# somepago/DCR

Hardware: NVIDIA H100
Metric: embed+top-k query images/sec (higher is better)
Workload: dtype bf16

## Files before the change

dcr_b200/csrc/stem_fused.cu:

```cuda
#include <cuda_bf16.h>

#include <algorithm>
#include <cstring>

#include "dcr_internal.cuh"
#include "host_util.cuh"
#include "ptx.cuh"

namespace dcr {

namespace {

constexpr int kSN = 64;
constexpr int kSTile = 512;
constexpr int kSBlocks = kSTile / 128;
constexpr int kSThreads = 288;
constexpr int kWBytes = kSN * 256 * 2;

struct StemParams {
  const __nv_bfloat16* planes;
  long long img_stride;
  long long plane_stride;
  int B, OH, OW, PW;
  int units_per_img, tiles_per_unit, num_units;
  int part_rows;
  int OHp, OWp, prow_per_part;
  int win_units;
  int win_stages;
  int ring_rows;
  const float* scale;
  const float* bias;
  __nv_bfloat16* out;
};

DCR_DEVICE uint64_t desc_nosw(uint32_t addr) {
  uint64_t d = 0;
  d |= static_cast<uint64_t>((addr & 0x3FFFF) >> 4);
  d |= static_cast<uint64_t>(16 >> 4) << 16;
  d |= static_cast<uint64_t>(256 >> 4) << 32;
  return d;
}

DCR_DEVICE void bulk_load(void* dst, const void* src, uint32_t bytes, uint64_t* bar) {
  asm volatile("cp.async.bulk.shared::cluster.global.mbarrier::complete_tx::bytes [%0], [%1], %2, [%3];" ::"r"(smem_u32(dst)),
               "l"(reinterpret_cast<uint64_t>(src)), "r"(bytes), "r"(smem_u32(bar))
               : "memory");
}

DCR_DEVICE int unit_begin(const StemParams& p, int part, bool pool) {
  if (!pool) return part * kSTile;
  const int row_lo = max(0, part * p.part_rows - 1);
  return row_lo * p.PW;
}

template <bool kPool>
__global__ void __launch_bounds__(kSThreads, 1) stem_conv_kernel(const __grid_constant__ CUtensorMap tmap_w, const StemParams p) {
  extern __shared__ __align__(1024) uint8_t smem_raw[];
  uint8_t* smem = smem_align1024(smem_raw);
  const int win_bytes = p.win_units * 16;
  const int stage_bytes = (2 * win_bytes + 1023) & ~1023;
  uint8_t* s_w = smem;
  uint8_t* s_win = s_w + kWBytes;
  uint8_t* s_out = s_win + p.win_stages * stage_bytes;
  const int ring_row_bytes = p.OW * 128;
  const int ring_mask = p.ring_rows - 1;
  uint8_t* acc_xpose = s_out + (kPool ? ((p.ring_rows * ring_row_bytes + 1023) & ~1023) : 2 * 16384);
  float* sb = reinterpret_cast<float*>(acc_xpose + 8 * kAccXposeWarpBytes);
  uint64_t* bars = reinterpret_cast<uint64_t*>(sb + 128);
  uint64_t* w_full = bars;
  uint64_t* win_full = bars + 1;
  uint64_t* win_empty = bars + 5;

  const uint32_t warp = threadIdx.x >> 5, lane = threadIdx.x & 31;
  if (warp == 8 && lane == 0) tma_prefetch_desc(&tmap_w);
  if (warp == 0 && lane == 0) {
    mbar_init(w_full, 1);
    for (int s = 0; s < 4; ++s) {
      mbar_init(&win_full[s], 1);
      mbar_init(&win_empty[s], 8);
    }
    fence_mbar_init();
  }
  __syncthreads();

  if (warp == 8) {
    if (elect_one()) {
      mbar_arrive_expect_tx(w_full, kWBytes);
      for (int kb = 0; kb < 4; ++kb) tma_load_2d(s_w + kb * 8192, &tmap_w, w_full, kb * 64, 0, kEvictLast);
    }
    __syncwarp();
    PipeState ws(p.win_stages);
    for (int unit = blockIdx.x; unit < p.num_units; unit += gridDim.x) {
      const int b = unit / p.units_per_img;
      const int mu = unit_begin(p, unit - b * p.units_per_img, kPool);
      for (int t = 0; t < p.tiles_per_unit; ++t, ws.next()) {
        const int m0 = mu + t * kSTile;
        mbar_wait(&win_empty[ws.s], ws.ph ^ 1);
        if (elect_one()) {
          mbar_arrive_expect_tx(&win_full[ws.s], 2 * win_bytes);
          const __nv_bfloat16* src = p.planes + static_cast<size_t>(b) * p.img_stride + static_cast<size_t>(m0) * 8;
          bulk_load(s_win + ws.s * stage_bytes, src, win_bytes, &win_full[ws.s]);
          bulk_load(s_win + ws.s * stage_bytes + win_bytes, src + p.plane_stride, win_bytes, &win_full[ws.s]);
        }
        __syncwarp();
      }
    }
  } else {
    const uint32_t ewarp = warp;
    const uint32_t quad = warp & 3;
    const uint32_t half = ewarp >> 2;
    const uint32_t row = quad * 32 + lane;
    const uint32_t etid = ewarp * 32 + lane;
    const uint32_t xacc = smem_u32(acc_xpose) + warp * kAccXposeWarpBytes;
    const uint32_t win0 = smem_u32(s_win);
    const uint32_t PW = static_cast<uint32_t>(p.PW);
    const uint64_t dw0 = wgmma_desc_sw128(smem_u32(s_w) + half * 32 * 128);
    PipeState ws(p.win_stages);
    const uint32_t sb_addr = smem_u32(sb), so_addr = smem_u32(s_out);
    for (int c = etid; c < kSN; c += 256) {
      st_shared_f32(sb_addr + c * 4, p.scale ? p.scale[c] : 1.f);
      st_shared_f32(sb_addr + (kSN + c) * 4, p.bias ? p.bias[c] : 0.f);
    }
    asm volatile("bar.sync 1, 256;" ::: "memory");
    float sc[32], bi[32];
#pragma unroll
    for (int c = 0; c < 32; c += 4) {
      const float4 s4 = ld_shared_f4(sb_addr + (half * 32 + c) * 4);
      const float4 b4 = ld_shared_f4(sb_addr + (kSN + half * 32 + c) * 4);
      sc[c] = s4.x; sc[c + 1] = s4.y; sc[c + 2] = s4.z; sc[c + 3] = s4.w;
      bi[c] = b4.x; bi[c + 1] = b4.y; bi[c + 2] = b4.z; bi[c + 3] = b4.w;
    }
    const int positions = p.OH * p.PW;
    mbar_wait(w_full, 0);
    uint32_t tc = 0, blk = 0;
    for (int unit = blockIdx.x; unit < p.num_units; unit += gridDim.x) {
      const int b = unit / p.units_per_img;
      const int part = unit - b * p.units_per_img;
      const int mu = unit_begin(p, part, kPool);
      const int row_lo = kPool ? max(0, part * p.part_rows - 1) : 0;
      const int row_hi = kPool ? min(p.OH, (part + 1) * p.part_rows) : p.OH;
      int next_yp = part * p.prow_per_part;
      const int yp_end = min(p.OHp, next_yp + p.prow_per_part);
      if constexpr (kPool) asm volatile("bar.sync 2, 256;" ::: "memory");
      for (int t = 0; t < p.tiles_per_unit; ++t, ++tc, ws.next()) {
        const int m0 = mu + t * kSTile;
        mbar_wait(&win_full[ws.s], ws.ph);
        const uint32_t wbase = win0 + ws.s * stage_bytes;
#pragma unroll 1
        for (int mb = 0; mb < kSBlocks; ++mb, ++blk) {
          WgAcc<32> acc;
          wgmma_fence();
#pragma unroll
          for (int a = 0; a < 4; ++a) {
#pragma unroll
            for (int e = 0; e < 2; ++e) {
#pragma unroll
              for (int bp = 0; bp < 2; ++bp) {
                const uint32_t a_addr = wbase + e * win_bytes + (mb * 128 + a * PW + 2 * bp) * 16;
                const int kc = (a * 2 + e) * 2 + bp;
                const uint64_t db = dw0 + static_cast<uint64_t>((kc >> 2) * (8192 >> 4) + (kc & 3) * 2);
                acc.mma2(desc_nosw(a_addr), desc_nosw(a_addr + 128), db, kc != 0);
              }
            }
          }
          wgmma_commit();
          wgmma_wait<0>();
          acc.fence_regs();
          if (mb == kSBlocks - 1 && lane == 0) mbar_arrive(&win_empty[ws.s]);
          uint32_t r[32];
          acc.rows32(0, r, xacc, lane);
          uint4 v[4];
#pragma unroll
          for (int q = 0; q < 4; ++q) {
            v[q].x = pack_bf16x2(fmaxf(fmaf(__uint_as_float(r[q * 8 + 0]), sc[q * 8 + 0], bi[q * 8 + 0]), 0.f),
                                 fmaxf(fmaf(__uint_as_float(r[q * 8 + 1]), sc[q * 8 + 1], bi[q * 8 + 1]), 0.f));
            v[q].y = pack_bf16x2(fmaxf(fmaf(__uint_as_float(r[q * 8 + 2]), sc[q * 8 + 2], bi[q * 8 + 2]), 0.f),
                                 fmaxf(fmaf(__uint_as_float(r[q * 8 + 3]), sc[q * 8 + 3], bi[q * 8 + 3]), 0.f));
            v[q].z = pack_bf16x2(fmaxf(fmaf(__uint_as_float(r[q * 8 + 4]), sc[q * 8 + 4], bi[q * 8 + 4]), 0.f),
                                 fmaxf(fmaf(__uint_as_float(r[q * 8 + 5]), sc[q * 8 + 5], bi[q * 8 + 5]), 0.f));
            v[q].w = pack_bf16x2(fmaxf(fmaf(__uint_as_float(r[q * 8 + 6]), sc[q * 8 + 6], bi[q * 8 + 6]), 0.f),
                                 fmaxf(fmaf(__uint_as_float(r[q * 8 + 7]), sc[q * 8 + 7], bi[q * 8 + 7]), 0.f));
          }
          const int mblk = m0 + mb * 128;
          if constexpr (!kPool) {
            const uint32_t stage = so_addr + (blk & 1) * 16384;
            const uint32_t srow = stage + row * 128;
            const uint32_t sw = row & 7;
#pragma unroll
            for (int q = 0; q < 4; ++q) st_shared_v4(srow + (((half * 4 + q) ^ sw) << 4), v[q]);
            asm volatile("bar.sync 2, 256;" ::: "memory");
#pragma unroll
            for (int it = 0; it < 4; ++it) {
              const int pos = it * 32 + static_cast<int>(etid >> 3);
              const int ch16 = static_cast<int>(etid & 7);
              const int m = mblk + pos;
              const int y = m / p.PW, x = m - y * p.PW;
              if (m < positions && x < p.OW) {
                const uint4 o = ld_shared_v4(stage + pos * 128 + ((ch16 ^ (pos & 7)) << 4));
                __nv_bfloat16* dst = p.out + ((static_cast<size_t>(b) * p.OH + y) * p.OW + x) * kSN + ch16 * 8;
                *reinterpret_cast<uint4*>(dst) = o;
              }
            }
          } else {
            const int m = mblk + static_cast<int>(row);
            const int y = m / p.PW, x = m - y * p.PW;
            if (x < p.OW && y >= row_lo && y < row_hi) {
              const uint32_t rrow = so_addr + (y & ring_mask) * ring_row_bytes + x * 128;
#pragma unroll
              for (int q = 0; q < 4; ++q) st_shared_v4(rrow + (((half * 4 + q) ^ (x & 7)) << 4), v[q]);
            }
            asm volatile("bar.sync 2, 256;" ::: "memory");
            const int yc = min((mblk + 128) / p.PW - 1, row_hi - 1);
            while (next_yp < yp_end && min(2 * next_yp + 1, p.OH - 1) <= yc) {
              const int y1 = 2 * next_yp;
              const uint32_t r0 = so_addr + (max(y1 - 1, 0) & ring_mask) * ring_row_bytes;
              const uint32_t r1 = so_addr + (y1 & ring_mask) * ring_row_bytes;
              const uint32_t r2 = so_addr + (min(y1 + 1, p.OH - 1) & ring_mask) * ring_row_bytes;
              for (int idx = etid; idx < p.OWp * 8; idx += 256) {
                const int xp = idx >> 3, c = idx & 7;
                const int x1 = 2 * xp, x0 = max(x1 - 1, 0), x2 = min(x1 + 1, p.OW - 1);
                const uint32_t o0 = x0 * 128 + ((c ^ (x0 & 7)) << 4), o1 = x1 * 128 + ((c ^ (x1 & 7)) << 4),
                               o2 = x2 * 128 + ((c ^ (x2 & 7)) << 4);
                uint4 w[9];
                w[0] = ld_shared_v4(r0 + o0); w[1] = ld_shared_v4(r0 + o1); w[2] = ld_shared_v4(r0 + o2);
                w[3] = ld_shared_v4(r1 + o0); w[4] = ld_shared_v4(r1 + o1); w[5] = ld_shared_v4(r1 + o2);
                w[6] = ld_shared_v4(r2 + o0); w[7] = ld_shared_v4(r2 + o1); w[8] = ld_shared_v4(r2 + o2);
                uint4 o;
                {
                  auto mx = [](uint32_t a, uint32_t b) {
                    __nv_bfloat162 r = __hmax2(*reinterpret_cast<const __nv_bfloat162*>(&a), *reinterpret_cast<const __nv_bfloat162*>(&b));
                    return *reinterpret_cast<uint32_t*>(&r);
                  };
                  auto mx9 = [&](auto get) {
                    const uint32_t a = mx(mx(get(w[0]), get(w[1])), mx(get(w[2]), get(w[3])));
                    const uint32_t b = mx(mx(get(w[4]), get(w[5])), mx(get(w[6]), get(w[7])));
                    return mx(mx(a, b), get(w[8]));
                  };
                  o.x = mx9([](const uint4& v) { return v.x; });
                  o.y = mx9([](const uint4& v) { return v.y; });
                  o.z = mx9([](const uint4& v) { return v.z; });
                  o.w = mx9([](const uint4& v) { return v.w; });
                }
                __nv_bfloat16* dst = p.out + ((static_cast<size_t>(b) * p.OHp + next_yp) * p.OWp + xp) * kSN + c * 8;
                *reinterpret_cast<uint4*>(dst) = o;
              }
              ++next_yp;
            }
          }
        }
      }
    }
  }

}

int stem_ring_rows(int PW) {
  int r = 8;
  while (r < 255 / PW + 4) r *= 2;
  return r;
}

}

int stem_fused_pitch(int out_w) { return out_w + 4; }
long long stem_fused_plane_units(int out_h, int out_w) {
  const int PW = stem_fused_pitch(out_w);
  const long long tiles = (static_cast<long long>(out_h) * PW + kSTile - 1) / kSTile;
  return tiles * kSTile + 3ll * PW + 16 + 2 * kSTile;
}

int stem_conv(const __nv_bfloat16* planes, int B, int OH, int OW, const __nv_bfloat16* weight, const float* scale, const float* bias,
              __nv_bfloat16* out, cudaStream_t stream, int pool) {
  const DeviceInfo* di = device_info();
  if (!di) return -2;
  if (int rc = require_sm90a(di, "stem_conv")) return rc;
  if (B == 0) return 0;
  StemParams p;
  memset(&p, 0, sizeof(p));
  p.planes = planes; p.B = B; p.OH = OH; p.OW = OW;
  p.PW = stem_fused_pitch(OW);
  p.plane_stride = stem_fused_plane_units(OH, OW) * 8;
  p.img_stride = 2 * p.plane_stride;
  const int tiles_per_img = static_cast<int>((static_cast<long long>(OH) * p.PW + kSTile - 1) / kSTile);
  p.win_units = (kSTile + 3 * p.PW + 3 + 7) & ~7;
  p.scale = scale; p.bias = bias; p.out = out;
  p.OHp = (OH - 1) / 2 + 1;
  p.OWp = (OW - 1) / 2 + 1;
  p.ring_rows = stem_ring_rows(p.PW);
  if (pool) {
    const int parts = (p.OHp % 4 == 0) ? 4 : ((p.OHp % 2 == 0) ? 2 : 1);
    p.units_per_img = parts;
    p.prow_per_part = p.OHp / parts;
    p.part_rows = 2 * p.prow_per_part;
    p.tiles_per_unit = static_cast<int>((static_cast<long long>(p.part_rows + 1) * p.PW + kSTile - 1) / kSTile);
    const long long last_unit = static_cast<long long>(std::max(0, (parts - 1) * p.part_rows - 1)) * p.PW;
    DCR_REQUIRE(last_unit + static_cast<long long>(p.tiles_per_unit) * kSTile + 3ll * p.PW + 8 <= stem_fused_plane_units(OH, OW),
                "stem_conv: plane slack too small for the pooled schedule (%d x %d)", OH, OW);
  } else {
    p.units_per_img = tiles_per_img;
    p.tiles_per_unit = 1;
    p.prow_per_part = 0;
    p.part_rows = 0;
  }
  p.num_units = B * p.units_per_img;
  CUtensorMap tw;
  if (int rc = make_tmap_2d_bf16(&tw, weight, kSN, 256, 256, kSN, 64)) return rc;
  const size_t stage = (static_cast<size_t>(2) * p.win_units * 16 + 1023) & ~size_t(1023);
  const size_t out_bytes = pool ? ((static_cast<size_t>(p.ring_rows) * OW * 128 + 1023) & ~size_t(1023)) : 2 * 16384;
  const size_t fixed = 1024 + kWBytes + out_bytes + 8 * kAccXposeWarpBytes + 512 + 256;
  DCR_REQUIRE(fixed + stage <= di->max_smem_optin, "stem_conv: image too wide for the window buffers (OW = %d)", OW);
  p.win_stages = static_cast<int>(std::min<size_t>(4, (di->max_smem_optin - fixed) / stage));
  const size_t smem = fixed + p.win_stages * stage;
  const int grid = std::min(p.num_units, di->num_sms);
  return launch(pool ? stem_conv_kernel<true> : stem_conv_kernel<false>, grid, kSThreads, smem, stream, "stem_conv", tw, p);
}

}
```

Baseline: 3459.

## Ping-pong two consumer warpgroups over full-width stem conv blocks

```diff
diff --git a/dcr_b200/csrc/stem_fused.cu b/dcr_b200/csrc/stem_fused.cu
--- a/dcr_b200/csrc/stem_fused.cu
+++ b/dcr_b200/csrc/stem_fused.cu
@@ -14,8 +14,11 @@
 constexpr int kSN = 64;
 constexpr int kSTile = 512;
 constexpr int kSBlocks = kSTile / 128;
-constexpr int kSThreads = 288;
+constexpr int kSThreads = 384;
+constexpr int kSConsumerRegs = 224, kSProducerRegs = 56;
 constexpr int kWBytes = kSN * 256 * 2;
+constexpr int kStageBytes = 128 * 128;
+constexpr int kSPoolMaxOW = 131;
 
 struct StemParams {
   const __nv_bfloat16* planes;
@@ -64,12 +67,13 @@
   uint8_t* s_out = s_win + p.win_stages * stage_bytes;
   const int ring_row_bytes = p.OW * 128;
   const int ring_mask = p.ring_rows - 1;
-  uint8_t* acc_xpose = s_out + (kPool ? ((p.ring_rows * ring_row_bytes + 1023) & ~1023) : 2 * 16384);
-  float* sb = reinterpret_cast<float*>(acc_xpose + 8 * kAccXposeWarpBytes);
-  uint64_t* bars = reinterpret_cast<uint64_t*>(sb + 128);
+  float* sb = reinterpret_cast<float*>(s_out + (kPool ? ((p.ring_rows * ring_row_bytes + 1023) & ~1023) : 2 * kStageBytes));
+  uint64_t* bars = reinterpret_cast<uint64_t*>(sb + 2 * kSN);
   uint64_t* w_full = bars;
   uint64_t* win_full = bars + 1;
   uint64_t* win_empty = bars + 5;
+  uint64_t* turn = bars + 9;
+  uint64_t* stored = bars + 11;
 
   const uint32_t warp = threadIdx.x >> 5, lane = threadIdx.x & 31;
   if (warp == 8 && lane == 0) tma_prefetch_desc(&tmap_w);
@@ -79,60 +83,67 @@
       mbar_init(&win_full[s], 1);
       mbar_init(&win_empty[s], 8);
     }
+    for (int g = 0; g < 2; ++g) {
+      mbar_init(&turn[g], 4);
+      mbar_init(&stored[g], 4);
+    }
     fence_mbar_init();
   }
   __syncthreads();
 
-  if (warp == 8) {
-    if (elect_one()) {
-      mbar_arrive_expect_tx(w_full, kWBytes);
-      for (int kb = 0; kb < 4; ++kb) tma_load_2d(s_w + kb * 8192, &tmap_w, w_full, kb * 64, 0, kEvictLast);
-    }
-    __syncwarp();
-    PipeState ws(p.win_stages);
-    for (int unit = blockIdx.x; unit < p.num_units; unit += gridDim.x) {
-      const int b = unit / p.units_per_img;
-      const int mu = unit_begin(p, unit - b * p.units_per_img, kPool);
-      for (int t = 0; t < p.tiles_per_unit; ++t, ws.next()) {
-        const int m0 = mu + t * kSTile;
-        mbar_wait(&win_empty[ws.s], ws.ph ^ 1);
-        if (elect_one()) {
-          mbar_arrive_expect_tx(&win_full[ws.s], 2 * win_bytes);
-          const __nv_bfloat16* src = p.planes + static_cast<size_t>(b) * p.img_stride + static_cast<size_t>(m0) * 8;
-          bulk_load(s_win + ws.s * stage_bytes, src, win_bytes, &win_full[ws.s]);
-          bulk_load(s_win + ws.s * stage_bytes + win_bytes, src + p.plane_stride, win_bytes, &win_full[ws.s]);
+  if (warp >= 8) {
+    wg_regs_dec<kSProducerRegs>();
+    if (warp == 8) {
+      if (elect_one()) {
+        mbar_arrive_expect_tx(w_full, kWBytes);
+        for (int kb = 0; kb < 4; ++kb) tma_load_2d(s_w + kb * 8192, &tmap_w, w_full, kb * 64, 0, kEvictLast);
+      }
+      __syncwarp();
+      PipeState ws(p.win_stages);
+      for (int unit = blockIdx.x; unit < p.num_units; unit += gridDim.x) {
+        const int b = unit / p.units_per_img;
+        const int mu = unit_begin(p, unit - b * p.units_per_img, kPool);
+        for (int t = 0; t < p.tiles_per_unit; ++t, ws.next()) {
+          const int m0 = mu + t * kSTile;
+          mbar_wait(&win_empty[ws.s], ws.ph ^ 1);
+          if (elect_one()) {
+            mbar_arrive_expect_tx(&win_full[ws.s], 2 * win_bytes);
+            const __nv_bfloat16* src = p.planes + static_cast<size_t>(b) * p.img_stride + static_cast<size_t>(m0) * 8;
+            bulk_load(s_win + ws.s * stage_bytes, src, win_bytes, &win_full[ws.s]);
+            bulk_load(s_win + ws.s * stage_bytes + win_bytes, src + p.plane_stride, win_bytes, &win_full[ws.s]);
+          }
+          __syncwarp();
         }
-        __syncwarp();
       }
     }
   } else {
-    const uint32_t ewarp = warp;
+    wg_regs_inc<kSConsumerRegs>();
+    const uint32_t wg = warp >> 2;
     const uint32_t quad = warp & 3;
-    const uint32_t half = ewarp >> 2;
-    const uint32_t row = quad * 32 + lane;
-    const uint32_t etid = ewarp * 32 + lane;
-    const uint32_t xacc = smem_u32(acc_xpose) + warp * kAccXposeWarpBytes;
+    const uint32_t gtid = quad * 32 + lane;
+    const uint32_t r0 = lane >> 2, c0 = 2 * (lane & 3);
     const uint32_t win0 = smem_u32(s_win);
     const uint32_t PW = static_cast<uint32_t>(p.PW);
-    const uint64_t dw0 = wgmma_desc_sw128(smem_u32(s_w) + half * 32 * 128);
-    PipeState ws(p.win_stages);
+    const uint64_t dw0 = wgmma_desc_sw128(smem_u32(s_w));
     const uint32_t sb_addr = smem_u32(sb), so_addr = smem_u32(s_out);
-    for (int c = etid; c < kSN; c += 256) {
+    for (int c = warp * 32 + lane; c < kSN; c += 256) {
       st_shared_f32(sb_addr + c * 4, p.scale ? p.scale[c] : 1.f);
       st_shared_f32(sb_addr + (kSN + c) * 4, p.bias ? p.bias[c] : 0.f);
     }
-    asm volatile("bar.sync 1, 256;" ::: "memory");
-    float sc[32], bi[32];
-#pragma unroll
-    for (int c = 0; c < 32; c += 4) {
-      const float4 s4 = ld_shared_f4(sb_addr + (half * 32 + c) * 4);
-      const float4 b4 = ld_shared_f4(sb_addr + (kSN + half * 32 + c) * 4);
-      sc[c] = s4.x; sc[c + 1] = s4.y; sc[c + 2] = s4.z; sc[c + 3] = s4.w;
-      bi[c] = b4.x; bi[c + 1] = b4.y; bi[c + 2] = b4.z; bi[c + 3] = b4.w;
+    named_bar_sync(1, 256);
+    float2 sc[8], bi[8];
+#pragma unroll
+    for (int j = 0; j < 8; ++j) {
+      sc[j] = ld_shared_f2(sb_addr + (8 * j + c0) * 4);
+      bi[j] = ld_shared_f2(sb_addr + (kSN + 8 * j + c0) * 4);
     }
     const int positions = p.OH * p.PW;
+    const PingPong pingpong{turn};
+    const PingPong ring_order{stored};
+    const uint32_t stage_addr = so_addr + wg * kStageBytes;
     mbar_wait(w_full, 0);
-    uint32_t tc = 0, blk = 0;
+    PipeState ws(p.win_stages);
+    uint32_t bc = 0;
     for (int unit = blockIdx.x; unit < p.num_units; unit += gridDim.x) {
       const int b = unit / p.units_per_img;
       const int part = unit - b * p.units_per_img;
@@ -141,14 +152,14 @@
       const int row_hi = kPool ? min(p.OH, (part + 1) * p.part_rows) : p.OH;
       int next_yp = part * p.prow_per_part;
       const int yp_end = min(p.OHp, next_yp + p.prow_per_part);
-      if constexpr (kPool) asm volatile("bar.sync 2, 256;" ::: "memory");
-      for (int t = 0; t < p.tiles_per_unit; ++t, ++tc, ws.next()) {
+      for (int t = 0; t < p.tiles_per_unit; ++t, ws.next()) {
         const int m0 = mu + t * kSTile;
         mbar_wait(&win_full[ws.s], ws.ph);
         const uint32_t wbase = win0 + ws.s * stage_bytes;
 #pragma unroll 1
-        for (int mb = 0; mb < kSBlocks; ++mb, ++blk) {
-          WgAcc<32> acc;
+        for (int mb = static_cast<int>(wg); mb < kSBlocks; mb += 2, ++bc) {
+          pingpong.wait(wg, bc);
+          WgAcc<kSN> acc;
           wgmma_fence();
 #pragma unroll
           for (int a = 0; a < 4; ++a) {
@@ -164,67 +175,70 @@
             }
           }
           wgmma_commit();
+          if (lane == 0) pingpong.hand_over(wg);
           wgmma_wait<0>();
           acc.fence_regs();
-          if (mb == kSBlocks - 1 && lane == 0) mbar_arrive(&win_empty[ws.s]);
-          uint32_t r[32];
-          acc.rows32(0, r, xacc, lane);
-          uint4 v[4];
-#pragma unroll
-          for (int q = 0; q < 4; ++q) {
-            v[q].x = pack_bf16x2(fmaxf(fmaf(__uint_as_float(r[q * 8 + 0]), sc[q * 8 + 0], bi[q * 8 + 0]), 0.f),
-                                 fmaxf(fmaf(__uint_as_float(r[q * 8 + 1]), sc[q * 8 + 1], bi[q * 8 + 1]), 0.f));
-            v[q].y = pack_bf16x2(fmaxf(fmaf(__uint_as_float(r[q * 8 + 2]), sc[q * 8 + 2], bi[q * 8 + 2]), 0.f),
-                                 fmaxf(fmaf(__uint_as_float(r[q * 8 + 3]), sc[q * 8 + 3], bi[q * 8 + 3]), 0.f));
-            v[q].z = pack_bf16x2(fmaxf(fmaf(__uint_as_float(r[q * 8 + 4]), sc[q * 8 + 4], bi[q * 8 + 4]), 0.f),
-                                 fmaxf(fmaf(__uint_as_float(r[q * 8 + 5]), sc[q * 8 + 5], bi[q * 8 + 5]), 0.f));
-            v[q].w = pack_bf16x2(fmaxf(fmaf(__uint_as_float(r[q * 8 + 6]), sc[q * 8 + 6], bi[q * 8 + 6]), 0.f),
-                                 fmaxf(fmaf(__uint_as_float(r[q * 8 + 7]), sc[q * 8 + 7], bi[q * 8 + 7]), 0.f));
-          }
+          if (mb + 2 >= kSBlocks && lane == 0) mbar_arrive(&win_empty[ws.s]);
           const int mblk = m0 + mb * 128;
           if constexpr (!kPool) {
-            const uint32_t stage = so_addr + (blk & 1) * 16384;
-            const uint32_t srow = stage + row * 128;
-            const uint32_t sw = row & 7;
-#pragma unroll
-            for (int q = 0; q < 4; ++q) st_shared_v4(srow + (((half * 4 + q) ^ sw) << 4), v[q]);
-            asm volatile("bar.sync 2, 256;" ::: "memory");
-#pragma unroll
-            for (int it = 0; it < 4; ++it) {
-              const int pos = it * 32 + static_cast<int>(etid >> 3);
-              const int ch16 = static_cast<int>(etid & 7);
+            named_bar_sync(2 + wg, 128);
+            acc.for_each_pair(lane, [&](uint32_t row, uint32_t col, float v0, float v1) {
+              const uint32_t j = (col - c0) >> 3;
+              const uint32_t v = pack_bf16x2(fmaxf(fmaf(v0, sc[j].x, bi[j].x), 0.f), fmaxf(fmaf(v1, sc[j].y, bi[j].y), 0.f));
+              st_shared_u32(stage_addr + (quad * 32 + row) * 128 + ((j ^ r0) << 4) + c0 * 2, v);
+            });
+            named_bar_sync(2 + wg, 128);
+#pragma unroll
+            for (int it = 0; it < 8; ++it) {
+              const int pos = it * 16 + static_cast<int>(gtid >> 3);
+              const int ch16 = static_cast<int>(gtid & 7);
               const int m = mblk + pos;
               const int y = m / p.PW, x = m - y * p.PW;
               if (m < positions && x < p.OW) {
-                const uint4 o = ld_shared_v4(stage + pos * 128 + ((ch16 ^ (pos & 7)) << 4));
+                const uint4 o = ld_shared_v4(stage_addr + pos * 128 + ((ch16 ^ (pos & 7)) << 4));
                 __nv_bfloat16* dst = p.out + ((static_cast<size_t>(b) * p.OH + y) * p.OW + x) * kSN + ch16 * 8;
                 *reinterpret_cast<uint4*>(dst) = o;
               }
             }
           } else {
-            const int m = mblk + static_cast<int>(row);
-            const int y = m / p.PW, x = m - y * p.PW;
-            if (x < p.OW && y >= row_lo && y < row_hi) {
-              const uint32_t rrow = so_addr + (y & ring_mask) * ring_row_bytes + x * 128;
-#pragma unroll
-              for (int q = 0; q < 4; ++q) st_shared_v4(rrow + (((half * 4 + q) ^ (x & 7)) << 4), v[q]);
-            }
-            asm volatile("bar.sync 2, 256;" ::: "memory");
+            if (t == 0 && mb == 0 && bc > 0) pingpong.wait(0, bc + 1);
+            uint32_t raddr[4], rsw[4];
+            bool rok[4];
+#pragma unroll
+            for (int g = 0; g < 4; ++g) {
+              const int m = mblk + static_cast<int>(quad * 32 + r0) + 8 * g;
+              const int y = m / p.PW, x = m - y * p.PW;
+              rok[g] = x < p.OW && y >= row_lo && y < row_hi;
+              raddr[g] = so_addr + (y & ring_mask) * ring_row_bytes + x * 128 + c0 * 2;
+              rsw[g] = static_cast<uint32_t>(x & 7);
+            }
+            acc.for_each_pair(lane, [&](uint32_t row, uint32_t col, float v0, float v1) {
+              const uint32_t g = (row - r0) >> 3, j = (col - c0) >> 3;
+              const uint32_t v = pack_bf16x2(fmaxf(fmaf(v0, sc[j].x, bi[j].x), 0.f), fmaxf(fmaf(v1, sc[j].y, bi[j].y), 0.f));
+              if (rok[g]) st_shared_u32(raddr[g] + ((j ^ rsw[g]) << 4), v);
+            });
+            named_bar_sync(2 + wg, 128);
+            ring_order.wait(wg, bc);
+            if (lane == 0) ring_order.hand_over(wg);
             const int yc = min((mblk + 128) / p.PW - 1, row_hi - 1);
+            if (t != 0 || mb != 0) {
+              const int yc_prev = min(mblk / p.PW - 1, row_hi - 1);
+              while (next_yp < yp_end && min(2 * next_yp + 1, p.OH - 1) <= yc_prev) ++next_yp;
+            }
             while (next_yp < yp_end && min(2 * next_yp + 1, p.OH - 1) <= yc) {
               const int y1 = 2 * next_yp;
-              const uint32_t r0 = so_addr + (max(y1 - 1, 0) & ring_mask) * ring_row_bytes;
-              const uint32_t r1 = so_addr + (y1 & ring_mask) * ring_row_bytes;
-              const uint32_t r2 = so_addr + (min(y1 + 1, p.OH - 1) & ring_mask) * ring_row_bytes;
-              for (int idx = etid; idx < p.OWp * 8; idx += 256) {
+              const uint32_t q0 = so_addr + (max(y1 - 1, 0) & ring_mask) * ring_row_bytes;
+              const uint32_t q1 = so_addr + (y1 & ring_mask) * ring_row_bytes;
+              const uint32_t q2 = so_addr + (min(y1 + 1, p.OH - 1) & ring_mask) * ring_row_bytes;
+              for (int idx = gtid; idx < p.OWp * 8; idx += 128) {
                 const int xp = idx >> 3, c = idx & 7;
                 const int x1 = 2 * xp, x0 = max(x1 - 1, 0), x2 = min(x1 + 1, p.OW - 1);
                 const uint32_t o0 = x0 * 128 + ((c ^ (x0 & 7)) << 4), o1 = x1 * 128 + ((c ^ (x1 & 7)) << 4),
                                o2 = x2 * 128 + ((c ^ (x2 & 7)) << 4);
                 uint4 w[9];
-                w[0] = ld_shared_v4(r0 + o0); w[1] = ld_shared_v4(r0 + o1); w[2] = ld_shared_v4(r0 + o2);
-                w[3] = ld_shared_v4(r1 + o0); w[4] = ld_shared_v4(r1 + o1); w[5] = ld_shared_v4(r1 + o2);
-                w[6] = ld_shared_v4(r2 + o0); w[7] = ld_shared_v4(r2 + o1); w[8] = ld_shared_v4(r2 + o2);
+                w[0] = ld_shared_v4(q0 + o0); w[1] = ld_shared_v4(q0 + o1); w[2] = ld_shared_v4(q0 + o2);
+                w[3] = ld_shared_v4(q1 + o0); w[4] = ld_shared_v4(q1 + o1); w[5] = ld_shared_v4(q1 + o2);
+                w[6] = ld_shared_v4(q2 + o0); w[7] = ld_shared_v4(q2 + o1); w[8] = ld_shared_v4(q2 + o2);
                 uint4 o;
                 {
                   auto mx = [](uint32_t a, uint32_t b) {
@@ -251,7 +265,6 @@
       }
     }
   }
-
 }
 
 int stem_ring_rows(int PW) {
@@ -274,6 +287,7 @@
   const DeviceInfo* di = device_info();
   if (!di) return -2;
   if (int rc = require_sm90a(di, "stem_conv")) return rc;
+  DCR_REQUIRE(!pool || OW <= kSPoolMaxOW, "stem_conv: image too wide for the pooling ring (OW = %d > %d)", OW, kSPoolMaxOW);
   if (B == 0) return 0;
   StemParams p;
   memset(&p, 0, sizeof(p));
@@ -306,8 +320,8 @@
   CUtensorMap tw;
   if (int rc = make_tmap_2d_bf16(&tw, weight, kSN, 256, 256, kSN, 64)) return rc;
   const size_t stage = (static_cast<size_t>(2) * p.win_units * 16 + 1023) & ~size_t(1023);
-  const size_t out_bytes = pool ? ((static_cast<size_t>(p.ring_rows) * OW * 128 + 1023) & ~size_t(1023)) : 2 * 16384;
-  const size_t fixed = 1024 + kWBytes + out_bytes + 8 * kAccXposeWarpBytes + 512 + 256;
+  const size_t out_bytes = pool ? ((static_cast<size_t>(p.ring_rows) * OW * 128 + 1023) & ~size_t(1023)) : 2 * kStageBytes;
+  const size_t fixed = 1024 + kWBytes + out_bytes + 512 + 256;
   DCR_REQUIRE(fixed + stage <= di->max_smem_optin, "stem_conv: image too wide for the window buffers (OW = %d)", OW);
   p.win_stages = static_cast<int>(std::min<size_t>(4, (di->max_smem_optin - fixed) / stage));
   const size_t smem = fixed + p.win_stages * stage;
```

Result: faster. 3508 (median of 6 runs) (+1.4%).

## Restructure stem conv as ping-pong warpgroups with register-resident weights

Applied to the files above, without the earlier changes.

```diff
diff --git a/dcr_b200/csrc/stem_fused.cu b/dcr_b200/csrc/stem_fused.cu
--- a/dcr_b200/csrc/stem_fused.cu
+++ b/dcr_b200/csrc/stem_fused.cu
@@ -14,8 +14,10 @@
 constexpr int kSN = 64;
 constexpr int kSTile = 512;
 constexpr int kSBlocks = kSTile / 128;
-constexpr int kSThreads = 288;
-constexpr int kWBytes = kSN * 256 * 2;
+constexpr int kSThreads = 384;
+constexpr int kSConsumerRegs = 224, kSProducerRegs = 56;
+constexpr int kSStageBytes = 128 * 128;
+constexpr int kSPoolMaxOW = 131;
 
 struct StemParams {
   const __nv_bfloat16* planes;
@@ -28,6 +30,7 @@
   int win_units;
   int win_stages;
   int ring_rows;
+  const __nv_bfloat16* weight;
   const float* scale;
   const float* bias;
   __nv_bfloat16* out;
@@ -37,8 +40,28 @@
   uint64_t d = 0;
   d |= static_cast<uint64_t>((addr & 0x3FFFF) >> 4);
   d |= static_cast<uint64_t>(16 >> 4) << 16;
-  d |= static_cast<uint64_t>(256 >> 4) << 32;
+  d |= static_cast<uint64_t>(128 >> 4) << 32;
   return d;
+}
+
+DCR_DEVICE void wgmma_m64n128_rs(float (&d)[64], const uint32_t (&a)[4], uint64_t db, uint32_t accumulate) {
+  asm volatile(
+      "{\n\t.reg .pred p;\n\t"
+      "setp.ne.b32 p, %68, 0;\n\t"
+      "wgmma.mma_async.sync.aligned.m64n128k16.f32.bf16.bf16 "
+      "{%0, %1, %2, %3, %4, %5, %6, %7, %8, %9, %10, %11, %12, %13, %14, %15, %16, %17, %18, %19, %20, %21, %22, %23, "
+      "%24, %25, %26, %27, %28, %29, %30, %31, %32, %33, %34, %35, %36, %37, %38, %39, %40, %41, %42, %43, %44, %45, "
+      "%46, %47, %48, %49, %50, %51, %52, %53, %54, %55, %56, %57, %58, %59, %60, %61, %62, %63}, "
+      "{%64, %65, %66, %67}, %69, p, 1, 1, 0;\n\t}\n"
+      : "+f"(d[0]), "+f"(d[1]), "+f"(d[2]), "+f"(d[3]), "+f"(d[4]), "+f"(d[5]), "+f"(d[6]), "+f"(d[7]), "+f"(d[8]),
+        "+f"(d[9]), "+f"(d[10]), "+f"(d[11]), "+f"(d[12]), "+f"(d[13]), "+f"(d[14]), "+f"(d[15]), "+f"(d[16]),
+        "+f"(d[17]), "+f"(d[18]), "+f"(d[19]), "+f"(d[20]), "+f"(d[21]), "+f"(d[22]), "+f"(d[23]), "+f"(d[24]),
+        "+f"(d[25]), "+f"(d[26]), "+f"(d[27]), "+f"(d[28]), "+f"(d[29]), "+f"(d[30]), "+f"(d[31]), "+f"(d[32]),
+        "+f"(d[33]), "+f"(d[34]), "+f"(d[35]), "+f"(d[36]), "+f"(d[37]), "+f"(d[38]), "+f"(d[39]), "+f"(d[40]),
+        "+f"(d[41]), "+f"(d[42]), "+f"(d[43]), "+f"(d[44]), "+f"(d[45]), "+f"(d[46]), "+f"(d[47]), "+f"(d[48]),
+        "+f"(d[49]), "+f"(d[50]), "+f"(d[51]), "+f"(d[52]), "+f"(d[53]), "+f"(d[54]), "+f"(d[55]), "+f"(d[56]),
+        "+f"(d[57]), "+f"(d[58]), "+f"(d[59]), "+f"(d[60]), "+f"(d[61]), "+f"(d[62]), "+f"(d[63])
+      : "r"(a[0]), "r"(a[1]), "r"(a[2]), "r"(a[3]), "r"(accumulate), "l"(db));
 }
 
 DCR_DEVICE void bulk_load(void* dst, const void* src, uint32_t bytes, uint64_t* bar) {
@@ -54,101 +77,94 @@
 }
 
 template <bool kPool>
-__global__ void __launch_bounds__(kSThreads, 1) stem_conv_kernel(const __grid_constant__ CUtensorMap tmap_w, const StemParams p) {
+__global__ void __launch_bounds__(kSThreads, 1) stem_conv_kernel(const StemParams p) {
   extern __shared__ __align__(1024) uint8_t smem_raw[];
   uint8_t* smem = smem_align1024(smem_raw);
   const int win_bytes = p.win_units * 16;
   const int stage_bytes = (2 * win_bytes + 1023) & ~1023;
-  uint8_t* s_w = smem;
-  uint8_t* s_win = s_w + kWBytes;
+  uint8_t* s_win = smem;
   uint8_t* s_out = s_win + p.win_stages * stage_bytes;
   const int ring_row_bytes = p.OW * 128;
   const int ring_mask = p.ring_rows - 1;
-  uint8_t* acc_xpose = s_out + (kPool ? ((p.ring_rows * ring_row_bytes + 1023) & ~1023) : 2 * 16384);
-  float* sb = reinterpret_cast<float*>(acc_xpose + 8 * kAccXposeWarpBytes);
-  uint64_t* bars = reinterpret_cast<uint64_t*>(sb + 128);
-  uint64_t* w_full = bars;
-  uint64_t* win_full = bars + 1;
-  uint64_t* win_empty = bars + 5;
+  uint64_t* bars = reinterpret_cast<uint64_t*>(s_out + (kPool ? ((p.ring_rows * ring_row_bytes + 1023) & ~1023) : 4 * kSStageBytes));
+  uint64_t* win_full = bars;
+  uint64_t* win_empty = bars + 4;
+  uint64_t* turn = bars + 8;
+  uint64_t* stored = bars + 10;
 
   const uint32_t warp = threadIdx.x >> 5, lane = threadIdx.x & 31;
-  if (warp == 8 && lane == 0) tma_prefetch_desc(&tmap_w);
   if (warp == 0 && lane == 0) {
-    mbar_init(w_full, 1);
     for (int s = 0; s < 4; ++s) {
       mbar_init(&win_full[s], 1);
       mbar_init(&win_empty[s], 8);
     }
+    for (int g = 0; g < 2; ++g) mbar_init(&turn[g], 4);
+    for (int s = 0; s < 4; ++s) mbar_init(&stored[s], 128);
     fence_mbar_init();
   }
   __syncthreads();
 
-  if (warp == 8) {
-    if (elect_one()) {
-      mbar_arrive_expect_tx(w_full, kWBytes);
-      for (int kb = 0; kb < 4; ++kb) tma_load_2d(s_w + kb * 8192, &tmap_w, w_full, kb * 64, 0, kEvictLast);
-    }
-    __syncwarp();
-    PipeState ws(p.win_stages);
-    for (int unit = blockIdx.x; unit < p.num_units; unit += gridDim.x) {
-      const int b = unit / p.units_per_img;
-      const int mu = unit_begin(p, unit - b * p.units_per_img, kPool);
-      for (int t = 0; t < p.tiles_per_unit; ++t, ws.next()) {
-        const int m0 = mu + t * kSTile;
-        mbar_wait(&win_empty[ws.s], ws.ph ^ 1);
-        if (elect_one()) {
-          mbar_arrive_expect_tx(&win_full[ws.s], 2 * win_bytes);
-          const __nv_bfloat16* src = p.planes + static_cast<size_t>(b) * p.img_stride + static_cast<size_t>(m0) * 8;
-          bulk_load(s_win + ws.s * stage_bytes, src, win_bytes, &win_full[ws.s]);
-          bulk_load(s_win + ws.s * stage_bytes + win_bytes, src + p.plane_stride, win_bytes, &win_full[ws.s]);
+  if (warp >= 8) {
+    wg_regs_dec<kSProducerRegs>();
+    if (warp == 8) {
+      PipeState ws(p.win_stages);
+      for (int unit = blockIdx.x; unit < p.num_units; unit += gridDim.x) {
+        const int b = unit / p.units_per_img;
+        const int mu = unit_begin(p, unit - b * p.units_per_img, kPool);
+        for (int t = 0; t < p.tiles_per_unit; ++t, ws.next()) {
+          const int m0 = mu + t * kSTile;
+          mbar_wait(&win_empty[ws.s], ws.ph ^ 1);
+          if (elect_one()) {
+            mbar_arrive_expect_tx(&win_full[ws.s], 2 * win_bytes);
+            const __nv_bfloat16* src = p.planes + static_cast<size_t>(b) * p.img_stride + static_cast<size_t>(m0) * 8;
+            bulk_load(s_win + ws.s * stage_bytes, src, win_bytes, &win_full[ws.s]);
+            bulk_load(s_win + ws.s * stage_bytes + win_bytes, src + p.plane_stride, win_bytes, &win_full[ws.s]);
+          }
+          __syncwarp();
         }
-        __syncwarp();
       }
     }
   } else {
-    const uint32_t ewarp = warp;
+    wg_regs_inc<kSConsumerRegs>();
+    const uint32_t wg = warp >> 2;
     const uint32_t quad = warp & 3;
-    const uint32_t half = ewarp >> 2;
-    const uint32_t row = quad * 32 + lane;
-    const uint32_t etid = ewarp * 32 + lane;
-    const uint32_t xacc = smem_u32(acc_xpose) + warp * kAccXposeWarpBytes;
+    const uint32_t gtid = quad * 32 + lane;
+    const uint32_t r0 = lane >> 2, c0 = 2 * (lane & 3);
     const uint32_t win0 = smem_u32(s_win);
     const uint32_t PW = static_cast<uint32_t>(p.PW);
-    const uint64_t dw0 = wgmma_desc_sw128(smem_u32(s_w) + half * 32 * 128);
+    const uint32_t so_addr = smem_u32(s_out);
+    const int ch = static_cast<int>(quad * 16 + r0);
+    uint32_t wa[16][4];
+#pragma unroll
+    for (int kc = 0; kc < 16; ++kc) {
+      const uint32_t* w0 = reinterpret_cast<const uint32_t*>(p.weight + ch * 256 + kc * 16 + c0);
+      const uint32_t* w1 = reinterpret_cast<const uint32_t*>(p.weight + (ch + 8) * 256 + kc * 16 + c0);
+      wa[kc][0] = w0[0]; wa[kc][1] = w1[0]; wa[kc][2] = w0[4]; wa[kc][3] = w1[4];
+    }
+    const float sc0 = p.scale ? p.scale[ch] : 1.f, sc1 = p.scale ? p.scale[ch + 8] : 1.f;
+    const float bi0 = p.bias ? p.bias[ch] : 0.f, bi1 = p.bias ? p.bias[ch + 8] : 0.f;
+    const uint32_t odd = r0 & 1;
+    const int positions = p.OH * p.PW;
+    const PingPong pingpong{turn};
     PipeState ws(p.win_stages);
-    const uint32_t sb_addr = smem_u32(sb), so_addr = smem_u32(s_out);
-    for (int c = etid; c < kSN; c += 256) {
-      st_shared_f32(sb_addr + c * 4, p.scale ? p.scale[c] : 1.f);
-      st_shared_f32(sb_addr + (kSN + c) * 4, p.bias ? p.bias[c] : 0.f);
-    }
-    asm volatile("bar.sync 1, 256;" ::: "memory");
-    float sc[32], bi[32];
-#pragma unroll
-    for (int c = 0; c < 32; c += 4) {
-      const float4 s4 = ld_shared_f4(sb_addr + (half * 32 + c) * 4);
-      const float4 b4 = ld_shared_f4(sb_addr + (kSN + half * 32 + c) * 4);
-      sc[c] = s4.x; sc[c + 1] = s4.y; sc[c + 2] = s4.z; sc[c + 3] = s4.w;
-      bi[c] = b4.x; bi[c + 1] = b4.y; bi[c + 2] = b4.z; bi[c + 3] = b4.w;
-    }
-    const int positions = p.OH * p.PW;
-    mbar_wait(w_full, 0);
-    uint32_t tc = 0, blk = 0;
+    uint32_t tc = 0;
+    int vbase = 0;
     for (int unit = blockIdx.x; unit < p.num_units; unit += gridDim.x) {
       const int b = unit / p.units_per_img;
       const int part = unit - b * p.units_per_img;
       const int mu = unit_begin(p, part, kPool);
       const int row_lo = kPool ? max(0, part * p.part_rows - 1) : 0;
       const int row_hi = kPool ? min(p.OH, (part + 1) * p.part_rows) : p.OH;
-      int next_yp = part * p.prow_per_part;
-      const int yp_end = min(p.OHp, next_yp + p.prow_per_part);
-      if constexpr (kPool) asm volatile("bar.sync 2, 256;" ::: "memory");
-      for (int t = 0; t < p.tiles_per_unit; ++t, ++tc, ws.next()) {
+      const int yp_begin = part * p.prow_per_part;
+      const int yp_end = min(p.OHp, yp_begin + p.prow_per_part);
+      for (int t = 0; t < p.tiles_per_unit; ++t, ws.next()) {
         const int m0 = mu + t * kSTile;
         mbar_wait(&win_full[ws.s], ws.ph);
         const uint32_t wbase = win0 + ws.s * stage_bytes;
 #pragma unroll 1
-        for (int mb = 0; mb < kSBlocks; ++mb, ++blk) {
-          WgAcc<32> acc;
+        for (int mb = wg; mb < kSBlocks; mb += 2, ++tc) {
+          pingpong.wait(wg, tc);
+          float acc[64];
           wgmma_fence();
 #pragma unroll
           for (int a = 0; a < 4; ++a) {
@@ -156,75 +172,89 @@
             for (int e = 0; e < 2; ++e) {
 #pragma unroll
               for (int bp = 0; bp < 2; ++bp) {
-                const uint32_t a_addr = wbase + e * win_bytes + (mb * 128 + a * PW + 2 * bp) * 16;
+                const uint32_t b_addr = wbase + e * win_bytes + (mb * 128 + a * PW + 2 * bp) * 16;
                 const int kc = (a * 2 + e) * 2 + bp;
-                const uint64_t db = dw0 + static_cast<uint64_t>((kc >> 2) * (8192 >> 4) + (kc & 3) * 2);
-                acc.mma2(desc_nosw(a_addr), desc_nosw(a_addr + 128), db, kc != 0);
+                wgmma_m64n128_rs(acc, wa[kc], desc_nosw(b_addr), kc != 0);
               }
             }
           }
           wgmma_commit();
+          if (lane == 0) pingpong.hand_over(wg);
           wgmma_wait<0>();
-          acc.fence_regs();
-          if (mb == kSBlocks - 1 && lane == 0) mbar_arrive(&win_empty[ws.s]);
-          uint32_t r[32];
-          acc.rows32(0, r, xacc, lane);
-          uint4 v[4];
-#pragma unroll
-          for (int q = 0; q < 4; ++q) {
-            v[q].x = pack_bf16x2(fmaxf(fmaf(__uint_as_float(r[q * 8 + 0]), sc[q * 8 + 0], bi[q * 8 + 0]), 0.f),
-                                 fmaxf(fmaf(__uint_as_float(r[q * 8 + 1]), sc[q * 8 + 1], bi[q * 8 + 1]), 0.f));
-            v[q].y = pack_bf16x2(fmaxf(fmaf(__uint_as_float(r[q * 8 + 2]), sc[q * 8 + 2], bi[q * 8 + 2]), 0.f),
-                                 fmaxf(fmaf(__uint_as_float(r[q * 8 + 3]), sc[q * 8 + 3], bi[q * 8 + 3]), 0.f));
-            v[q].z = pack_bf16x2(fmaxf(fmaf(__uint_as_float(r[q * 8 + 4]), sc[q * 8 + 4], bi[q * 8 + 4]), 0.f),
-                                 fmaxf(fmaf(__uint_as_float(r[q * 8 + 5]), sc[q * 8 + 5], bi[q * 8 + 5]), 0.f));
-            v[q].w = pack_bf16x2(fmaxf(fmaf(__uint_as_float(r[q * 8 + 6]), sc[q * 8 + 6], bi[q * 8 + 6]), 0.f),
-                                 fmaxf(fmaf(__uint_as_float(r[q * 8 + 7]), sc[q * 8 + 7], bi[q * 8 + 7]), 0.f));
+#pragma unroll
+          for (int i = 0; i < 64; ++i) asm volatile("" : "+f"(acc[i])::"memory");
+          if (mb + 2 >= kSBlocks && lane == 0) mbar_arrive(&win_empty[ws.s]);
+          const int mblk = m0 + mb * 128;
+          const int pos0 = static_cast<int>(c0 + odd);
+          int y = (mblk + pos0) / p.PW, x = mblk + pos0 - y * p.PW;
+#pragma unroll
+          for (int j = 0; j < 16; ++j) {
+            const int pos = pos0 + 8 * j;
+            uint32_t dst, swz;
+            bool valid;
+            if constexpr (kPool) {
+              valid = x < p.OW && y >= row_lo && y < row_hi;
+              dst = so_addr + ((vbase + y - row_lo) & ring_mask) * ring_row_bytes + x * 128;
+              swz = x & 7;
+            } else {
+              valid = true;
+              dst = so_addr + (wg * 2 + (tc & 1)) * kSStageBytes + pos * 128;
+              swz = pos & 7;
+            }
+#pragma unroll
+            for (int h = 0; h < 2; ++h) {
+              const float s = h ? sc1 : sc0, t = h ? bi1 : bi0;
+              const float v0 = fmaxf(fmaf(acc[4 * j + 2 * h], s, t), 0.f);
+              const float v1 = fmaxf(fmaf(acc[4 * j + 2 * h + 1], s, t), 0.f);
+              const float got = __shfl_xor_sync(0xffffffffu, odd ? v0 : v1, 4);
+              const uint32_t v = odd ? pack_bf16x2(got, v1) : pack_bf16x2(v0, got);
+              const uint32_t chunk = quad * 2 + h;
+              if (valid) st_shared_u32(dst + ((chunk ^ swz) << 4) + (r0 >> 1) * 4, v);
+            }
+            x += 8;
+            while (x >= p.PW) {
+              x -= p.PW;
+              ++y;
+            }
           }
-          const int mblk = m0 + mb * 128;
           if constexpr (!kPool) {
-            const uint32_t stage = so_addr + (blk & 1) * 16384;
-            const uint32_t srow = stage + row * 128;
-            const uint32_t sw = row & 7;
-#pragma unroll
-            for (int q = 0; q < 4; ++q) st_shared_v4(srow + (((half * 4 + q) ^ sw) << 4), v[q]);
-            asm volatile("bar.sync 2, 256;" ::: "memory");
-#pragma unroll
-            for (int it = 0; it < 4; ++it) {
-              const int pos = it * 32 + static_cast<int>(etid >> 3);
-              const int ch16 = static_cast<int>(etid & 7);
+            named_bar_sync(2 + wg, 128);
+            const uint32_t stage = so_addr + (wg * 2 + (tc & 1)) * kSStageBytes;
+#pragma unroll
+            for (int it = 0; it < 8; ++it) {
+              const int pos = it * 16 + static_cast<int>(gtid >> 3);
+              const int ch16 = static_cast<int>(gtid & 7);
               const int m = mblk + pos;
               const int y = m / p.PW, x = m - y * p.PW;
               if (m < positions && x < p.OW) {
                 const uint4 o = ld_shared_v4(stage + pos * 128 + ((ch16 ^ (pos & 7)) << 4));
-                __nv_bfloat16* dst = p.out + ((static_cast<size_t>(b) * p.OH + y) * p.OW + x) * kSN + ch16 * 8;
-                *reinterpret_cast<uint4*>(dst) = o;
+                __nv_bfloat16* out = p.out + ((static_cast<size_t>(b) * p.OH + y) * p.OW + x) * kSN + ch16 * 8;
+                *reinterpret_cast<uint4*>(out) = o;
               }
             }
           } else {
-            const int m = mblk + static_cast<int>(row);
-            const int y = m / p.PW, x = m - y * p.PW;
-            if (x < p.OW && y >= row_lo && y < row_hi) {
-              const uint32_t rrow = so_addr + (y & ring_mask) * ring_row_bytes + x * 128;
-#pragma unroll
-              for (int q = 0; q < 4; ++q) st_shared_v4(rrow + (((half * 4 + q) ^ (x & 7)) << 4), v[q]);
-            }
-            asm volatile("bar.sync 2, 256;" ::: "memory");
+            mbar_arrive(&stored[wg * 2 + (tc & 1)]);
+            named_bar_sync(2 + wg, 128);
+            if (wg == 1) mbar_wait(&stored[0 * 2 + (tc & 1)], (tc >> 1) & 1);
+            else if (tc > 0) mbar_wait(&stored[1 * 2 + ((tc - 1) & 1)], ((tc - 1) >> 1) & 1);
             const int yc = min((mblk + 128) / p.PW - 1, row_hi - 1);
-            while (next_yp < yp_end && min(2 * next_yp + 1, p.OH - 1) <= yc) {
-              const int y1 = 2 * next_yp;
-              const uint32_t r0 = so_addr + (max(y1 - 1, 0) & ring_mask) * ring_row_bytes;
-              const uint32_t r1 = so_addr + (y1 & ring_mask) * ring_row_bytes;
-              const uint32_t r2 = so_addr + (min(y1 + 1, p.OH - 1) & ring_mask) * ring_row_bytes;
-              for (int idx = etid; idx < p.OWp * 8; idx += 256) {
+            const int yc_prev = min(mblk / p.PW - 1, row_hi - 1);
+            auto last_row = [&](int yp) { return min(2 * yp + 1, p.OH - 1); };
+            for (int yp = max(yp_begin, (yc_prev + 1) >> 1); yp < yp_end && last_row(yp) <= yc; ++yp) {
+              if (last_row(yp) <= yc_prev) continue;
+              const int y1 = 2 * yp;
+              const uint32_t r0a = so_addr + ((vbase + max(y1 - 1, 0) - row_lo) & ring_mask) * ring_row_bytes;
+              const uint32_t r1a = so_addr + ((vbase + y1 - row_lo) & ring_mask) * ring_row_bytes;
+              const uint32_t r2a = so_addr + ((vbase + min(y1 + 1, p.OH - 1) - row_lo) & ring_mask) * ring_row_bytes;
+              for (int idx = gtid; idx < p.OWp * 8; idx += 128) {
                 const int xp = idx >> 3, c = idx & 7;
                 const int x1 = 2 * xp, x0 = max(x1 - 1, 0), x2 = min(x1 + 1, p.OW - 1);
                 const uint32_t o0 = x0 * 128 + ((c ^ (x0 & 7)) << 4), o1 = x1 * 128 + ((c ^ (x1 & 7)) << 4),
                                o2 = x2 * 128 + ((c ^ (x2 & 7)) << 4);
                 uint4 w[9];
-                w[0] = ld_shared_v4(r0 + o0); w[1] = ld_shared_v4(r0 + o1); w[2] = ld_shared_v4(r0 + o2);
-                w[3] = ld_shared_v4(r1 + o0); w[4] = ld_shared_v4(r1 + o1); w[5] = ld_shared_v4(r1 + o2);
-                w[6] = ld_shared_v4(r2 + o0); w[7] = ld_shared_v4(r2 + o1); w[8] = ld_shared_v4(r2 + o2);
+                w[0] = ld_shared_v4(r0a + o0); w[1] = ld_shared_v4(r0a + o1); w[2] = ld_shared_v4(r0a + o2);
+                w[3] = ld_shared_v4(r1a + o0); w[4] = ld_shared_v4(r1a + o1); w[5] = ld_shared_v4(r1a + o2);
+                w[6] = ld_shared_v4(r2a + o0); w[7] = ld_shared_v4(r2a + o1); w[8] = ld_shared_v4(r2a + o2);
                 uint4 o;
                 {
                   auto mx = [](uint32_t a, uint32_t b) {
@@ -241,22 +271,21 @@
                   o.z = mx9([](const uint4& v) { return v.z; });
                   o.w = mx9([](const uint4& v) { return v.w; });
                 }
-                __nv_bfloat16* dst = p.out + ((static_cast<size_t>(b) * p.OHp + next_yp) * p.OWp + xp) * kSN + c * 8;
-                *reinterpret_cast<uint4*>(dst) = o;
+                __nv_bfloat16* out = p.out + ((static_cast<size_t>(b) * p.OHp + yp) * p.OWp + xp) * kSN + c * 8;
+                *reinterpret_cast<uint4*>(out) = o;
               }
-              ++next_yp;
             }
           }
         }
       }
+      if constexpr (kPool) vbase += row_hi - row_lo;
     }
   }
-
 }
 
 int stem_ring_rows(int PW) {
   int r = 8;
-  while (r < 255 / PW + 4) r *= 2;
+  while (r < 383 / PW + 4) r *= 2;
   return r;
 }
 
@@ -303,16 +332,16 @@
     p.part_rows = 0;
   }
   p.num_units = B * p.units_per_img;
-  CUtensorMap tw;
-  if (int rc = make_tmap_2d_bf16(&tw, weight, kSN, 256, 256, kSN, 64)) return rc;
+  p.weight = weight;
   const size_t stage = (static_cast<size_t>(2) * p.win_units * 16 + 1023) & ~size_t(1023);
-  const size_t out_bytes = pool ? ((static_cast<size_t>(p.ring_rows) * OW * 128 + 1023) & ~size_t(1023)) : 2 * 16384;
-  const size_t fixed = 1024 + kWBytes + out_bytes + 8 * kAccXposeWarpBytes + 512 + 256;
+  const size_t out_bytes = pool ? ((static_cast<size_t>(p.ring_rows) * OW * 128 + 1023) & ~size_t(1023)) : 4 * kSStageBytes;
+  const size_t fixed = 1024 + out_bytes + 256;
+  DCR_REQUIRE(!pool || OW <= kSPoolMaxOW, "stem_conv: image too wide for the pooled stem (OW = %d > %d)", OW, kSPoolMaxOW);
   DCR_REQUIRE(fixed + stage <= di->max_smem_optin, "stem_conv: image too wide for the window buffers (OW = %d)", OW);
   p.win_stages = static_cast<int>(std::min<size_t>(4, (di->max_smem_optin - fixed) / stage));
   const size_t smem = fixed + p.win_stages * stage;
   const int grid = std::min(p.num_units, di->num_sms);
-  return launch(pool ? stem_conv_kernel<true> : stem_conv_kernel<false>, grid, kSThreads, smem, stream, "stem_conv", tw, p);
-}
-
-}
+  return launch(pool ? stem_conv_kernel<true> : stem_conv_kernel<false>, grid, kSThreads, smem, stream, "stem_conv", p);
+}
+
+}
```

After: 3446 before, 3496 after (median of 6 runs). +1.5%, better.
